# CodeKnight314/Goal-Conditioned-RL-Framework

Measured on AMD Instinct MI355X. Metric: gradient-steps/sec (HER sample + critic+actor update), higher is better.
Workload: dtype f32; 1 GPU; ddpg_pickplace_b256; agent=DDPG, batch_per_gpu=256, buffer_rows=1000000, state_dim=23, action_dim=4, hidden=256, layers=3, k_future=8, gradient_step=40, parallelism=single, hip_graph=True, rng=cpython-mt19937 (host) indices

## Files before the change

### goal-conditioned-rl-framework_amd/_ffi.py

```python
from __future__ import annotations

import ctypes as C
import os

_HERE = os.path.dirname(os.path.abspath(__file__))
LIB_PATH = os.environ.get("GCRL_HIP_LIB") or os.path.join(_HERE, "libgcrl_hip.so")

STREAM_LEGACY = 1
CLONE_AGENT, CLONE_RING = 1, 2
XCHG_HANDLE_BYTES = 256


class GcrlError(RuntimeError):
    pass


class NotEnoughSamples(AssertionError):
    """len(buffer) < batch_size — the reference asserts (src/buffer.py:122)."""


class HerConfig(C.Structure):
    _fields_ = [
        ("state_dim", C.c_int32), ("action_dim", C.c_int32), ("goal_dim", C.c_int32),
        ("capacity", C.c_int64), ("nenvs", C.c_int32), ("k_future", C.c_int32),
# ... 161 lines not shown
    "gcrl_tanh_gauss_bwd_f32": (C.c_int, [_vp, C.c_int, C.c_int, _vp, C.c_int, _vp, _vp, _vp, C.c_int, _f32, C.c_int, C.c_int, _vp, _vp,
                                          C.c_int, _vp]),
    "gcrl_actor_select_f32": (C.c_int, [_vp, _vp, _f32, C.c_int, C.c_int, C.c_int, C.c_int, C.c_int, _f32, _f32, C.c_int, _vp, _vp, _vp, _vp]),
    "gcrl_td3_smooth_f32": (C.c_int, [_vp, C.c_int, C.c_int, C.c_int, _vp, _f32, _f32, _vp]),
    "gcrl_her_set_reward_callback": (C.c_int, [_vp, _vp, _vp]),
    "gcrl_agent_dp_sync_bn": (C.c_int, [_vp, C.c_int, C.c_int, _vp, _vp, _vp]),
    "gcrl_agent_bn_xchg_create": (_vp, [_vp, C.c_int, C.c_int]),
    "gcrl_agent_dp_sync_bn_xchg": (C.c_int, [_vp, C.c_int, C.c_int, _vp]),
    "gcrl_xchg_create": (_vp, [_vp, _i64, _vp, _vp, C.c_int, C.c_int, C.c_int, C.c_int]),
    "gcrl_xchg_destroy": (None, [_vp]),
    "gcrl_xchg_handles": (C.c_int, [_vp, _vp, _i64]),
    "gcrl_xchg_connect": (C.c_int, [_vp, _vp, _i64]),
    "gcrl_xchg_world": (C.c_int, [_vp]),
    "gcrl_xchg_allreduce": (C.c_int, [_vp, C.c_int, C.c_int, _vp]),
    "gcrl_xchg_reset": (C.c_int, [_vp]),
    "gcrl_xchg_selftest": (C.c_int, [_vp, _vp]),
    "gcrl_xchg_read": (C.c_int, [_vp, _i64, _i64, _vp]),
    "gcrl_xchg_get_partials": (C.c_int, [_vp, C.c_int, _vp, C.c_int]),
    "gcrl_agent_xchg_create": (_vp, [_vp, C.c_int, C.c_int]),
    "gcrl_agent_set_exchange": (C.c_int, [_vp, _vp]),
    "gcrl_set_shared_device": (C.c_int, [C.c_int]),
    "gcrl_agent_set_meetings": (C.c_int, [_vp, C.c_int]),
    "gcrl_agent_get_meetings": (C.c_int, [_vp]),
    "gcrl_agent_debug_meet_fault": (C.c_int, [_vp]),
    "gcrl_hash_normal_fill": (C.c_int, [C.c_uint64, C.c_uint64, C.c_int64, _vp, _vp]),
    "gcrl_event_create": (_vp, []),
    "gcrl_event_destroy": (None, [_vp]),
    "gcrl_event_record": (C.c_int, [_vp, _vp]),
    "gcrl_event_elapsed_ms": (C.c_int, [_vp, _vp, C.POINTER(_f32)]),
    "gcrl_stream_synchronize": (C.c_int, [_vp]),
    "gcrl_malloc": (_vp, [C.c_size_t]),
    "gcrl_free": (None, [_vp]),
    "gcrl_memcpy_h2d": (C.c_int, [_vp, _vp, C.c_size_t, _vp]),
    "gcrl_memcpy_d2h": (C.c_int, [_vp, _vp, C.c_size_t, _vp]),
}


def _load():
    if not os.path.exists(LIB_PATH):
        raise ImportError(
            f"{LIB_PATH} is missing: build the HIP extension first "
            "(python -c 'import __graft_entry__ as g; g.build()' or make -C csrc). "
            "There is no CPU fallback.")
    import torch
    lib = C.CDLL(LIB_PATH)
    for name, (res, args) in PROTOTYPES.items():
# ... 43 lines not shown
```

### goal-conditioned-rl-framework_amd/csrc/agent.hip

```cpp
#include <hip/hip_runtime.h>

#include <algorithm>
#include <cmath>
#include <cstdlib>
#include <map>
#include <mutex>
#include <random>
#include <string>
#include <vector>

#include "act_bn.h"
#include "dw_adam.h"
#include "gemm_mfma.h"
#include "her_ring.h"
#include "meet.h"
#include "ops.h"
#include "rowchain.h"
#include "sac_heads.h"
#include "xchg_ipc.h"
#include "pop.h"
#include "pbt_host.h"

using namespace gcrl;

// ... 1948 lines not shown
  for (auto& kv : a->graphs) (void)hipGraphExecDestroy(kv.second);
  a->graphs.clear();
  const gcrl_agent_config& c = a->cfg;
  const bool want = on != 0 && !meet_device_shared();
  a->bn_rsplit = (want && a->bn_slab && a->B > 128 && !std::getenv("GCRL_NO_BN_RSPLIT") && bn_slab_row_split(a->B, a->H, 2) > 1) ? 4 : 1;
  a->rc_merge = want && a->rc_bar && a->split_roles && !std::getenv("GCRL_NO_RC_MERGE") && !std::getenv("GCRL_SPLIT_RG") &&
                rowchain_merge_ok(a->row_rg, a->row_ldl, c.ac_dim, a->H, a->C, a->B);
  a->rc_merge_k = want && a->rc_bar && a->split_k && !std::getenv("GCRL_NO_RC_MERGE");
  a->ddpg_ksplit = want && a->ddpg_ksplit_can && a->rc_bar && !std::getenv("GCRL_NO_DDPG_KSPLIT");
  a->rowtile = want && a->rowtile_can && rowtile_enabled() && rowtile_ok(a->B, a->H, a->L, a->S, a->A, a->C);
  a->opt_fuse = want && a->opt_fuse_can && !std::getenv("GCRL_NO_OPT_FUSE");
  return (a->bn_rsplit > 1 ? 1 : 0) | ((a->rc_merge || a->rc_merge_k || a->ddpg_ksplit) ? 2 : 0) | (a->rowtile ? 4 : 0) | (a->opt_fuse ? 8 : 0);
}

int gcrl_agent_get_meetings(gcrl_agent* a) {
  GCRL_CHECK_ARG(a, "gcrl_agent_get_meetings: null handle");
  if (!meet_device_shared() && meet_probe_device(a->cfg.device)) {
    const int rc = gcrl_agent_set_meetings(a, 0);
    if (rc < 0) return rc;
  }
  return (a->bn_rsplit > 1 ? 1 : 0) | ((a->rc_merge || a->rc_merge_k || a->ddpg_ksplit) ? 2 : 0) | (a->rowtile ? 4 : 0) | (a->opt_fuse ? 8 : 0);
}

int gcrl_agent_debug_meet_fault(gcrl_agent* a) {
  GCRL_CHECK_ARG(a, "gcrl_agent_debug_meet_fault: null handle");
  GCRL_HIP(hipDeviceSynchronize());
  const unsigned long long one = 7;
  float* words = a->rc_merge ? a->rc_bar : (a->bn_rsplit > 1 ? a->bn_bar : nullptr);
  if (a->rowtile) {
    GCRL_HIP(hipMemcpy(a->rt_ctr, &one, sizeof(one), hipMemcpyHostToDevice));
    return GCRL_OK;
  }
  if (a->rc_merge_k || (a->ddpg_ksplit && !a->rowtile)) {
    const unsigned long long far = 1ull << 40;
    GCRL_HIP(hipMemcpy(a->rc_bar + 4, &far, sizeof(far), hipMemcpyHostToDevice));
    return GCRL_OK;
  }
  if (a->opt_fuse) {
    const unsigned int on = 1;
    GCRL_HIP(hipMemcpy(reinterpret_cast<unsigned int*>(a->of_seq) + 1, &on, sizeof(on), hipMemcpyHostToDevice));
    return GCRL_OK;
  }
  GCRL_CHECK_ARG(words, "gcrl_agent_debug_meet_fault: this agent's launches contain no waits (meetings off or not applicable)");
  if (words == a->bn_bar && bn_slab_data_flag()) {
    const unsigned int on = 1;
    GCRL_HIP(hipMemcpy(reinterpret_cast<unsigned int*>(a->bn_bar) + 1, &on, sizeof(on), hipMemcpyHostToDevice));
// ... 314 lines not shown
```

### goal-conditioned-rl-framework_amd/csrc/agent_pop.inc

```

struct gcrl_pop {
  std::vector<gcrl_agent*> m;
  std::map<std::string, void*> tabs;
  std::vector<PopRec> rec;
  long long want[3] = {0, 0, 0}, cap[3] = {0, 0, 0};
  bool no_waits = false;
  int64_t merged = 0, alone = 0;
  bool gather_merge = false;
  int64_t upd_calls = 0, gather_merged = 0, gather_alone = 0;
  PopTabCache act_tabs;
  char *act_blk_host = nullptr, *act_blk_dev = nullptr;
  unsigned long long act_seq = 0;
  char *act_st_host = nullptr, *act_st_dev = nullptr;
  std::vector<int64_t> act_ordered;
  PopProcStep proc;
  int64_t act_calls = 0, act_launches = 0, act_staged = 0;
  PopTabCache clone_tabs;
};

namespace {

constexpr int kMaxPopMembers = 16;
constexpr int kPopActRows = 32;

// ... 319 lines not shown
  };
  const int chunk = std::min(kMaxStepsPerCall, a0->Mmax);
  for (int done = 0; done < n; done += chunk) {
    const int m = std::min(chunk, n - done);
    std::vector<std::vector<StepPlan>> plans(P);
    CallGather cgs[kMaxPopMembers];
    for (int i = 0; i < P; ++i) {
      gcrl_agent* a = p->m[i];
      if (a->wt_dirty) TRY(rc_rebuild_wt(a, st));
      TRY(begin_call_plan(a, rings[i], step0 + done, m, nullptr, 1.0f, st, plans[i], tickets_out ? tickets_out + (size_t)i * n + done : nullptr,
                          tuple_len_out ? tuple_len_out + (size_t)i * n + done : nullptr, false, !tqc || pop_layer_adv(a),
                          &cgs[i]));
    }
    bool one = false;
    TRY(begin_call_issue_pop(p->m.data(), cgs, P, p->gather_merge, st, &one));
    p->upd_calls++;
    if (one) p->gather_merged++;
    else p->gather_alone += P;
    int rc = GCRL_OK;
    for (int i = 0; i < P && !rc; ++i) {
      gcrl_agent* a = p->m[i];
      a->ddpg_ksplit = ksplit; a->opt_fuse = ofuse; a->rowtile = false;
      if (sac) { a->rc_merge = merge; if (!rsplit) a->bn_rsplit = 1; }
      rc = pop_record_steps(a, a0->cap_stream, plans[i], &p->rec[i]);
    }
    restore();
    if (rc) return rc;
    const size_t K = p->rec[0].ops.size();
    for (int i = 1; i < P; ++i)
      if (p->rec[i].ops.size() != K) return fail(GCRL_ERR_STATE, "gcrl_pop_update_n: member %d's step has %zu launches, member 0's %zu", i, p->rec[i].ops.size(), K);
    for (size_t k = 0; k < K; ++k) TRY(pop_issue(p, k, st));
    for (gcrl_agent* a : p->m) TRY(end_call(a, st));
  }
  return GCRL_OK;
}

int gcrl_pop_observe_act(gcrl_pop* p, gcrl_normalizer* const* nz_obs, gcrl_normalizer* const* nz_dg, const float* obs_host, int32_t obs_dim,
                         const float* dg_host, int32_t goal_dim, int32_t n, const double* noise_host, const int32_t* modes, double* out_host,
                         void* stream) {
  GCRL_CHECK_ARG(obs_host, "gcrl_pop_observe_act: obs_host: null array");
  GCRL_CHECK_ARG(dg_host, "gcrl_pop_observe_act: dg_host: null array");
  GCRL_CHECK_ARG(modes, "gcrl_pop_observe_act: modes: null array");
  GCRL_CHECK_ARG(out_host, "gcrl_pop_observe_act: out_host: null array");
  GCRL_CHECK_ARG(modes[0] >= -1 && modes[0] <= 2, "gcrl_pop_observe_act: modes: member 0 has mode %d (-1 skipped, 0, 1 or 2)", modes[0]);
  GCRL_CHECK_ARG(p, "gcrl_pop_observe_act: pop: null handle");
  const int P = (int)p->m.size();
// ... 397 lines not shown
```

### goal-conditioned-rl-framework_amd/csrc/pop.h

```cpp
#pragma once

#include <hip/hip_runtime.h>

#include <atomic>
#include <cstring>
#include <functional>
#include <map>
#include <string>
#include <utility>
#include <vector>

namespace gcrl {

enum PopKind {
  POP_ALONE = 0,
  POP_ROWCHAIN = 1,
  POP_DW_ADAM = 2,
  POP_BEGIN_STEP = 3,
  POP_GEMM_BATCH = 4,
  POP_ADAM = 5,
  POP_ADAM_PAIR = 6,
  POP_BN_FWD = 7,
  POP_BN_BWD = 8,
  POP_BN_BWD_FOLD = 9,
  POP_RC_SPLIT = 10,
  POP_RC_SPLIT_HEADS = 11,
  POP_TG_BWD_SELECT = 12,
  POP_TG_FWD = 13,
  POP_TG_BWD = 14,
};
inline bool pop_mergeable(int kind, int sub) { return kind != POP_ALONE && (kind != POP_GEMM_BATCH || sub == 1); }

struct PopOp {
  int kind = POP_ALONE;
  int sub = 0;
  dim3 grid;
  size_t lds = 0;
  std::vector<char> args;
  std::function<int(hipStream_t)> issue;
};

struct PopRec {
  std::vector<PopOp> ops;
};

PopRec*& pop_rec();
extern std::atomic<int> g_pop_recorders;
inline PopRec* pop_recording() { return g_pop_recorders.load(std::memory_order_relaxed) ? pop_rec() : nullptr; }

inline int pop_record(PopRec* r, int kind, int sub, dim3 grid, size_t lds, const void* args, size_t bytes,
                      std::function<int(hipStream_t)> issue) {
  PopOp op;
  op.kind = kind; op.sub = sub; op.grid = grid; op.lds = lds;
  if (bytes) { op.args.resize(bytes); std::memcpy(op.args.data(), args, bytes); }
  op.issue = std::move(issue);
  r->ops.push_back(std::move(op));
  return 0;
}
inline int pop_defer(PopRec* r, std::function<int(hipStream_t)> issue) {
  return pop_record(r, POP_ALONE, 0, dim3(1), 0, nullptr, 0, std::move(issue));
}

struct PopTabCache {
  std::map<std::string, void*> tabs;
  const std::string* last = nullptr;
  void* last_dev = nullptr;
// ... 45 lines not shown
```

### goal-conditioned-rl-framework_amd/csrc/rowchain.h

```cpp
#pragma once
#include <hip/hip_runtime.h>

#include "gemm_mfma.h"
#include "ops.h"

namespace gcrl {

constexpr int kRowThreads = 256;
constexpr int kRowChunk = 256;

__device__ inline __amdgpu_buffer_rsrc_t bounded_rsrc(const float* p, long long nfloats) {
  const unsigned long long v = (unsigned long long)p;
  const unsigned int lo = __builtin_amdgcn_readfirstlane((unsigned int)v);
  const unsigned int hi = __builtin_amdgcn_readfirstlane((unsigned int)(v >> 32));
  void* q = (void*)(((unsigned long long)hi << 32) | lo);
  const int bytes = __builtin_amdgcn_readfirstlane((int)(nfloats * 4));
  return __builtin_amdgcn_make_buffer_rsrc(q, 0, bytes, 0x00020000);
}

template <int RG>
__device__ __forceinline__ void rows_matmul_wave(const float* xs, int ldx, __amdgpu_buffer_rsrc_t rs, int ldm, int c0,
                                        int jb, int je, v4f (&acc)[RG][4]) {
  const int lane = threadIdx.x & 63;
  constexpr int U = 8;
// ... 14 lines not shown
#pragma unroll
        for (int g = 0; g < RG; ++g) xa[g] = *(const v4f*)(xs + (4 * g + (lane & 3)) * ldx + j + u4);
#pragma unroll
        for (int u = 0; u < 4; ++u)
#pragma unroll
          for (int q = 0; q < 4; ++q)
#pragma unroll
            for (int g = 0; g < RG; ++g)
              acc[g][q] = __builtin_amdgcn_mfma_f32_4x4x1f32(xa[g][u], __uint_as_float(w[u4 + u][q]), acc[g][q], 0, 0, 0);
      }
    }
  };
  v4u wa[U], wb[U];
  load(wa, jb);
  for (int j = jb; j < je; j += 2 * U) {
    load(wb, j + U);
    compute(wa, j);
    load(wa, j + 2 * U);
    compute(wb, j + U);
  }
}

template <int RG>
__device__ __forceinline__ void rows_linear(const float* xs, int ldx, int J, const float* M, int ldm, int N, const float* bias,
                                   int epi, float* part, float* ys, int ldy, float* save, long long ld_save,
                                   int rows_valid, const float* mulH = nullptr, long long ld_mul = 0, int mul = MUL_NONE,
                                   bool chained = false, int pbuf = 0) {
  constexpr int R = 4 * RG;
  const int lane = threadIdx.x & 63;
  const int wave = __builtin_amdgcn_readfirstlane(threadIdx.x >> 6);
  const __amdgpu_buffer_rsrc_t rs = bounded_rsrc(M, (long long)J * ldm);
  const int per = ((J + 3) / 4 + 3) & ~3;
  const int jb = wave * per, je = min(J, jb + per);
  if (chained) {
    part += pbuf * (4 * R * kRowChunk);
    const int pern = ((N + 3) / 4 + 3) & ~3, q4 = pern >> 2;
    const int cb = wave * pern;
    v4f eb[RG], eh[RG];
#pragma unroll
    for (int it = 0; it < RG; ++it) {
      const int idx = lane + 64 * it, r = idx / q4, cc = cb + 4 * (idx - r * q4);
      const bool ok = idx < R * q4 && cc < N;
      eb[it] = (bias && ok) ? *(const v4f*)(bias + cc) : (v4f){0.f, 0.f, 0.f, 0.f};
      eh[it] = (mulH && ok && r < rows_valid) ? *(const v4f*)(mulH + (long long)r * ld_mul + cc) : (v4f){0.f, 0.f, 0.f, 0.f};
    }
    v4f acc[RG][4];
    rows_matmul_wave<RG>(xs, ldx, rs, ldm, 0, jb, je, acc);
#pragma unroll
    for (int g = 0; g < RG; ++g)
#pragma unroll
      for (int i = 0; i < 4; ++i)
        *(v4f*)(part + ((wave * R + 4 * g + i) * kRowChunk) + 4 * lane) =
            (v4f){acc[g][0][i], acc[g][1][i], acc[g][2][i], acc[g][3][i]};
    __syncthreads();
#pragma unroll
    for (int it = 0; it < RG; ++it) {
      const int idx = lane + 64 * it, r = idx / q4, cc = cb + 4 * (idx - r * q4);
      if (idx < R * q4 && cc < N) {
        v4f v = *(const v4f*)(part + r * kRowChunk + cc);
#pragma unroll
        for (int w = 1; w < 4; ++w) v += *(const v4f*)(part + (w * R + r) * kRowChunk + cc);
        v += eb[it];
#pragma unroll
        for (int q = 0; q < 4; ++q) {
          v[q] = act_apply(v[q], epi);
          if (mul != MUL_NONE) v[q] *= act_deriv(eh[it][q], mul);
        }
        *(v4f*)(ys + r * ldy + cc) = v;
        if (save && r < rows_valid) *(v4f*)(save + (long long)r * ld_save + cc) = v;
      }
    }
    return;
  }
  for (int c0 = 0; c0 < N; c0 += kRowChunk) {
    const int c = c0 + 4 * lane;
    v4f b = (v4f){0.f, 0.f, 0.f, 0.f}, hm[RG];
    if (bias && c < N) b = *(const v4f*)(bias + c);
#pragma unroll
    for (int rr = 0; rr < RG; ++rr) {
      const int r = wave + 4 * rr;
      hm[rr] = (mulH && c < N && r < rows_valid) ? *(const v4f*)(mulH + (long long)r * ld_mul + c) : (v4f){0.f, 0.f, 0.f, 0.f};
    }
    v4f acc[RG][4];
    rows_matmul_wave<RG>(xs, ldx, rs, ldm, c0, jb, je, acc);
#pragma unroll
    for (int g = 0; g < RG; ++g)
#pragma unroll
      for (int i = 0; i < 4; ++i)
        *(v4f*)(part + ((wave * R + 4 * g + i) * kRowChunk) + 4 * lane) =
            (v4f){acc[g][0][i], acc[g][1][i], acc[g][2][i], acc[g][3][i]};
    __syncthreads();
    if (c < N) {
#pragma unroll
      for (int rr = 0; rr < RG; ++rr) {
        const int r = wave + 4 * rr;
        v4f v = *(const v4f*)(part + (0 * R + r) * kRowChunk + 4 * lane);
#pragma unroll
        for (int w = 1; w < 4; ++w) v += *(const v4f*)(part + (w * R + r) * kRowChunk + 4 * lane);
        v += b;
#pragma unroll
        for (int q = 0; q < 4; ++q) {
          v[q] = act_apply(v[q], epi);
          if (mul != MUL_NONE) v[q] *= act_deriv(hm[rr][q], mul);
        }
        *(v4f*)(ys + r * ldy + c) = v;
        if (save && r < rows_valid) *(v4f*)(save + (long long)r * ld_save + c) = v;
      }
// ... 47 lines not shown
  const StepCtrl* cur_k; const StepCtrl* cur_p;
  CtrlBlock* cb;
  RowNet actor, tactor, critic[2], tcritic[2];
  int C;
  int target_kind, loss_kind;
  const float* noise; float policy_noise, noise_clamp; unsigned long long seed;
  int given_next, p_critic_only;
  const float* logp_next; float alpha;
  const float* pi;
  const float* sa; const float* nsa; const float* rbuf; const float* dbuf;
  long long slot_x, slot_rd;
  int ldx, ldl, B, S, A, Apad;
  int nblk_k, nblk_p;
  int linear_roles;
  float *hC, *gC, *q, *y, *dq;
  float *hA, *gA, *hC2, *q2, *dz;
  float gamma, clamp_lo;
  unsigned long long* clk;
  float* qt;
  unsigned int* bar;
  unsigned int* status;
  int producers_first;
  int k_split;
};

struct HeadsFold {
  int on;
  int cur_in_k;
  const float* P;
  long long w_mean, b_mean, w_ls, b_ls;
  const float* h_next; const float* h_cur;
  const float* eps_next; const float* eps_cur;
  float* logp_next;
  float* pi; float* logp; float* save_eps; float* save_std; float* head;
  BnRunning run;
};
int launch_rowchain_split(hipStream_t st, const RowChainArgs& a, int rg, int phase, int part, const HeadsFold* hf = nullptr);
bool rowchain_merge_ok(int rg, int ldl, int A, int H, int C, int B);

struct RowActArgs {
  RowNet actor;
  const float* obs; int ld_obs;
  float* out; int ld_out;
  int n, S, A, ldl;
  const double* nz_mean; const double* nz_var; double nz_clip; int D;
  const double* nzg_mean; const double* nzg_var; double nzg_clip;
// ... 20 lines not shown
  unsigned int live, noisy;
  int stride_n;
};
int launch_rowchain_act_pop(hipStream_t st, const RowActPop& c, int members, int n, int ldl, int A, int H);

struct RowTileArgs {
  RowChainArgs rc;
  float* xb;
  float* qpart;
  unsigned long long* ctr;
  unsigned int* xid;
  unsigned int* status;
  int force_sc1;
  int roles[3], nroles, nstage, w16, ldsx, kperx, force_linear, role_mask, sleep_first, sleep_poll;
};
bool rowtile_shape_ok(int B, int H, int L, int S, int A, int C);
bool rowtile_ok(int B, int H, int L, int S, int A, int C);
long long rowtile_ctr_words(int B, int L);
long long rowtile_xb_floats(int B, int H, int L);
long long rowtile_part_floats(int B, int H);
int launch_rowtile_ddpg(hipStream_t st, RowTileArgs t);

int launch_rowchain_ddpg(hipStream_t st, const RowChainArgs& a, int rg);
size_t rowchain_lds_bytes(int rg, int ldl, int A, int H, int C);

int launch_wt_rebuild(hipStream_t st, const RowNet& net, float* Wt);

}
```

### goal-conditioned-rl-framework_amd/csrc/rowchain.hip

```cpp
#include "rowchain.h"
#include "norm_math.h"
#include "meet.h"
#include "sac_select.h"
#include "pop.h"

#include <algorithm>

namespace gcrl {
namespace {

template <int RG>
__device__ inline void load_rows(float* X, int ldl, const float* src, long long ld_src, int ncols, int jpad, int rv) {
  constexpr int R = 4 * RG;
  for (int i = threadIdx.x; i < R * jpad; i += kRowThreads) {
    const int r = i / jpad, c = i - r * jpad;
    X[r * ldl + c] = (r < rv && c < ncols) ? src[(long long)r * ld_src + c] : 0.f;
  }
}

template <int RG>
__device__ inline float* mlp_hidden(const RowNet& net, const float* X0, float* X1, float* X2, int ldl, float* part,
                                    float* save, long long BH, long long row0, int rv, float* last_out = nullptr) {
  const float* in = X0;
  float* out = X1;
  const bool chained = RG == 1 && net.H <= kRowChunk;
  for (int l = 0; l < net.L; ++l) {
    if (last_out && l == net.L - 1) out = last_out;
    rows_linear<RG>(in, ldl, l == 0 ? net.jpad0 : net.H, net.Wt + net.wt[l], net.H, net.H, net.P + net.b[l], EPI_LEAKY,
                    part, out, ldl, save ? save + l * BH + row0 * net.H : nullptr, net.H, rv, nullptr, 0, MUL_NONE,
                    chained, l & 1);
    in = out;
    out = (out == X1) ? X2 : X1;
  }
  if (chained) __syncthreads();
  return (float*)in;
}

template <int RG>
__device__ inline void head_backward(float* h, int ldl, int H, const float* Wh, int n_up, const float* up ,
                                     float* save, int rv, float* q_out = nullptr, float q_bias = 0.f) {
  constexpr int R = 4 * RG;
  const int H4 = H >> 2;
  for (int i = threadIdx.x; i < R * H4; i += kRowThreads) {
    const int r = i / H4, k = (i - r * H4) << 2;
    const v4f hv = *(const v4f*)(h + r * ldl + k);
    v4f s = (v4f){0.f, 0.f, 0.f, 0.f};
    for (int o = 0; o < n_up; ++o) s += up[r * 16 + o] * *(const v4f*)(Wh + (long long)o * H + k);
    v4f g;
#pragma unroll
    for (int q = 0; q < 4; ++q) g[q] = s[q] * act_deriv(hv[q], MUL_DLEAKY);
    if (q_out) {
      const v4f w = *(const v4f*)(Wh + k);
      float qs = ((hv[0] * w[0] + hv[1] * w[1]) + hv[2] * w[2]) + hv[3] * w[3];
// ... 35 lines not shown
#pragma unroll
  for (int u = 0; u < N; ++u) { const int i = threadIdx.x + u * kRowThreads; if (i < n) dst[i] = s.v[u]; }
  for (int i = threadIdx.x + N * kRowThreads; i < n; i += kRowThreads) dst[i] = src[i];
}
template <int RG, int N>
__device__ inline void rows_load(Staged<N>& s, const float* src, long long ld_src, int ncols, int jpad, int rv) {
#pragma unroll
  for (int u = 0; u < N; ++u) {
    const int i = threadIdx.x + u * kRowThreads, r = i / jpad, c = i - r * jpad;
    s.v[u] = (i < 4 * RG * jpad && r < rv && c < ncols) ? src[(long long)r * ld_src + c] : 0.f;
  }
}
template <int RG, int N>
__device__ inline void rows_store(const Staged<N>& s, float* X, int ldl, const float* src, long long ld_src, int ncols, int jpad, int rv) {
#pragma unroll
  for (int u = 0; u < N; ++u) {
    const int i = threadIdx.x + u * kRowThreads, r = i / jpad, c = i - r * jpad;
    if (i < 4 * RG * jpad) X[r * ldl + c] = s.v[u];
  }
  for (int i = threadIdx.x + N * kRowThreads; i < 4 * RG * jpad; i += kRowThreads) {
    const int r = i / jpad, c = i - r * jpad;
    X[r * ldl + c] = (r < rv && c < ncols) ? src[(long long)r * ld_src + c] : 0.f;
  }
}

__device__ inline void stage(float* dst, const float* src, int n) {
  for (int i0 = threadIdx.x; i0 < n; i0 += 8 * kRowThreads) {
    float v[8];
#pragma unroll
    for (int u = 0; u < 8; ++u) { const int i = i0 + u * kRowThreads; v[u] = i < n ? src[i] : 0.f; }
#pragma unroll
    for (int u = 0; u < 8; ++u) { const int i = i0 + u * kRowThreads; if (i < n) dst[i] = v[u]; }
  }
}

template <int RG, bool HF = false>
__device__ __forceinline__ void rowchain_split_body(const RowChainArgs& a, int phase, int part, int bid, const HeadsFold& hfr = HeadsFold{});

template <int RG>
__global__ __launch_bounds__(kRowThreads) void rowchain_ddpg_kernel(RowChainArgs a) {
  kernarg_warm<sizeof(RowChainArgs)>();
#include "rowchain_ddpg_body.inc"
}

template <int RG>
__global__ __launch_bounds__(kRowThreads) void rowchain_ddpg_pop_kernel(const RowChainArgs* __restrict__ tab) {
// ... 428 lines not shown
  const float* rows = c.rows + (size_t)m * c.stride_n * a.ld_obs;
  const double* noise = c.noise + (size_t)m * c.stride_n * a.A;
  double* out = c.out + (size_t)m * c.stride_n * a.A;
  rowchain_act_body<true>(a, [&](long long i) { return __hip_atomic_load(rows + i, __ATOMIC_RELAXED, __HIP_MEMORY_SCOPE_SYSTEM); },
                          [&](long long t) { return __hip_atomic_load(noise + t, __ATOMIC_RELAXED, __HIP_MEMORY_SCOPE_SYSTEM); },
                          ((c.noisy >> m) & 1u) != 0, out, lds);
  asm volatile("s_waitcnt vmcnt(0)" ::: "memory");
  __syncthreads();
  if (threadIdx.x == 0 && c.flags) __hip_atomic_store(c.flags + (size_t)m * gridDim.x + blockIdx.x, c.seq, __ATOMIC_RELAXED, __HIP_MEMORY_SCOPE_SYSTEM);
}

__global__ void wt_rebuild_kernel(RowNet net, float* Wt) {
  const int l = blockIdx.y;
  const int in = l == 0 ? net.in : net.H, J = l == 0 ? net.jpad0 : net.H, H = net.H;
  const long long n = (long long)J * H;
  for (long long i = (long long)blockIdx.x * blockDim.x + threadIdx.x; i < n; i += (long long)gridDim.x * blockDim.x) {
    const int k = (int)(i / H), o = (int)(i - (long long)k * H);
    Wt[net.wt[l] + i] = k < in ? net.P[net.w[l] + (long long)o * in + k] : 0.f;
  }
}

}

size_t rowchain_lds_bytes(int rg, int ldl, int A, int H, int C) {
  const int R = 4 * rg;
  return (size_t)(4 * R * ldl + (rg == 1 ? 2 : 1) * 4 * R * kRowChunk + 4 * R * 16 + std::max(std::max(2 * A + 1, A + 2 * C), C * (A + 1)) * H + 96) * sizeof(float);
}

bool rowchain_merge_ok(int rg, int ldl, int A, int H, int C, int B) {
  const size_t lds = rowchain_lds_bytes(rg, ldl, A, H, C);
  if (lds > 160 * 1024) return false;
  const void* k = rg == 1 ? (const void*)rowchain_split_kernel<1> : (rg == 2 ? (const void*)rowchain_split_kernel<2> : (const void*)rowchain_split_kernel<4>);
  if (lds > 64 * 1024 && hipFuncSetAttribute(k, hipFuncAttributeMaxDynamicSharedMemorySize, (int)lds) != hipSuccess) return false;
  const long long nblk = (B + 4 * rg - 1) / (4 * rg);
  const void* kh = rg == 1 ? (const void*)rowchain_split_heads_kernel<1> : (rg == 2 ? (const void*)rowchain_split_heads_kernel<2> : (const void*)rowchain_split_heads_kernel<4>);
  if (lds > 64 * 1024 && hipFuncSetAttribute(kh, hipFuncAttributeMaxDynamicSharedMemorySize, (int)lds) != hipSuccess) return false;
  return 2LL * C * nblk <= meet_capacity(k, kRowThreads, lds) && 2LL * C * nblk <= meet_capacity(kh, kRowThreads, lds);
}

int launch_rowchain_ddpg(hipStream_t st, const RowChainArgs& a, int rg) {
  GCRL_CHECK_ARG(rg == 1 || rg == 2 || rg == 4, "rowchain: rows per block must be 4, 8 or 16");
  GCRL_CHECK_ARG(a.critic[0].H % 4 == 0 && a.ldl % 4 == 0 && a.A <= 16 && a.C >= 1 && a.C <= 2,
                 "rowchain: unsupported shape (H=%d, A=%d, C=%d)", a.critic[0].H, a.A, a.C);
  const size_t lds = rowchain_lds_bytes(rg, a.ldl, a.A, a.critic[0].H, a.C);
  GCRL_CHECK_ARG(lds <= 160 * 1024, "rowchain: %zu bytes of LDS needed", lds);
  GCRL_CHECK_ARG(!a.k_split || (a.bar && a.qt && a.producers_first && a.C == 1), "rowchain: the two-role critic phase needs its meeting counters");
  const int grid = (a.k_split ? 2 : 1) * a.nblk_k + a.nblk_p;
  if (grid < 1) return GCRL_OK;
  if (PopRec* r = pop_recording())
    return pop_record(r, POP_ROWCHAIN, rg, dim3(grid), lds, &a, sizeof(a), [ac = a, rg](hipStream_t s) { return launch_rowchain_ddpg(s, ac, rg); });
  auto go = [&](auto kern) -> int {
    static thread_local size_t raised = 0;
    if (lds > 64 * 1024 && lds > raised) {
      GCRL_HIP(hipFuncSetAttribute((const void*)kern, hipFuncAttributeMaxDynamicSharedMemorySize, (int)lds));
      raised = lds;
    }
    hipLaunchKernelGGL(kern, dim3(grid), dim3(kRowThreads), lds, st, a);
    GCRL_HIP(hipGetLastError());
    return GCRL_OK;
  };
  if (rg == 1) return go(rowchain_ddpg_kernel<1>);
  if (rg == 2) return go(rowchain_ddpg_kernel<2>);
  return go(rowchain_ddpg_kernel<4>);
}

int launch_rowchain_split(hipStream_t st, const RowChainArgs& a, int rg, int phase, int part, const HeadsFold* hf) {
  GCRL_CHECK_ARG(rg == 1 || rg == 2 || rg == 4, "rowchain: rows per block must be 4, 8 or 16");
  GCRL_CHECK_ARG(a.critic[0].H % 4 == 0 && a.ldl % 4 == 0 && a.A <= 16 && a.C >= 1 && a.C <= 2 && (phase == 0 || phase == 1) &&
                     (part >= 1 && part <= 3) && (part != 3 || a.bar) && (phase == 0 || a.p_critic_only) && a.qt,
                 "rowchain split: unsupported shape (H=%d, A=%d, C=%d, phase %d part %d)", a.critic[0].H, a.A, a.C, phase, part);
  const size_t lds = rowchain_lds_bytes(rg, a.ldl, a.A, a.critic[0].H, a.C);
  GCRL_CHECK_ARG(lds <= 160 * 1024, "rowchain: %zu bytes of LDS needed", lds);
  const int nblk = (a.B + 4 * rg - 1) / (4 * rg);
// ... 154 lines not shown
```

### goal-conditioned-rl-framework_amd/csrc/rowchain_ddpg_body.inc

```
  extern __shared__ __attribute__((aligned(16))) float lds[];
  if (a.k_split && a.nblk_k) {
    if ((int)blockIdx.x < 2 * a.nblk_k) {
      if (a.clk && threadIdx.x == 0 && blockIdx.x == 0) atomicMin(&a.clk[0], (unsigned long long)wall_clock64());
      rowchain_split_body<RG>(a, 0, 3, (int)blockIdx.x);
      if (a.clk && threadIdx.x == 0) atomicMax(&a.clk[1], (unsigned long long)wall_clock64());
      return;
    }
  }
  const int kblocks = (a.k_split && a.nblk_k) ? 2 * a.nblk_k : a.nblk_k;
  constexpr int R = 4 * RG;
  const int ldl = a.ldl, H = a.critic[0].H, S = a.S, A = a.A, B = a.B;
  float* X0 = lds;
  float* X1 = X0 + R * ldl;
  float* X2 = X1 + R * ldl;
  float* XS = X2 + R * ldl;
  float* part = XS + R * ldl;
  float* sm = part + R * 16 + (RG == 1 ? 2 : 1) * 4 * R * kRowChunk;
  float* sm2 = sm + R * 16;
  float* sm3 = sm2 + R * 16;
  float* hw = sm3 + R * 16;
  float* hb = hw + max(max(2 * A + 1, A + 2 * a.C), a.C * (A + 1)) * H;
  bool role_k = (int)blockIdx.x < kblocks;
  int blk = role_k ? (int)blockIdx.x : (int)blockIdx.x - kblocks;
  if (a.nblk_k == a.nblk_p && (a.nblk_k & 3) == 0 && !a.linear_roles && !a.k_split) {
// ... 142 lines not shown
      if (r < rv) { a.q2[row0 + r] = q0; if (C > 1) a.q2[(long long)B + row0 + r] = q1; }
    }
    __syncthreads();
    for (int k = 0; k < C; ++k) {
      const float* hs = a.hC2 + (long long)k * a.critic[k].L * BH;
      const float* hsrc = hs + (a.critic[k].L - 1) * BH + row0 * H;
      for (int i = tid; i < R * H; i += kRowThreads) {
        const int r = i / H, kk = i - r * H;
        XS[r * ldl + kk] = r < rv ? hsrc[(long long)r * H + kk] : 0.f;
      }
      __syncthreads();
      head_backward<RG>(XS, ldl, H, hw_c + k * H, 1, sm2 + k, nullptr, rv);
      __syncthreads();
      float* g0 = grad_chain<RG>(a.critic[k], XS, X1, X2, ldl, part + R * 16, hs, nullptr, BH, row0, rv);
      rows_head<RG>(g0, ldl, H, hw_da + k * A * H, H, nullptr, A, EPI_NONE, sm);
      __syncthreads();
      if (tid < R * A) {
        const int r = tid / A, o = tid - r * A;
        if (r < rv) a.dz[((long long)k * B + row0 + r) * a.Apad + o] = sm[r * 16 + o];
      }
      __syncthreads();
    }
  } else {
    const StepCtrl c = *a.cur_p;
    const float* sa_rows = a.sa + (long long)c.batch_slot * a.slot_x + row0 * a.ldx;
    constexpr int NX = 2 * RG;
    const int jp_s = max(a.actor.jpad0, a.critic[0].jpad0);
    float* hw_a = hw; float* hw_c = hw + A * H; float* hw_da = hw_c + H;
    const float* src_a = a.actor.P + a.actor.w[a.actor.L];
    const float* src_c = a.critic[0].P + a.critic[0].w[a.critic[0].L];
    const float* src_da = a.critic[0].Wt + a.critic[0].wt[0] + (long long)S * H;
    Staged<NX> s_s;
    rows_load<RG>(s_s, sa_rows, a.ldx, S, jp_s, rv);
    Staged<8> s_a, s_hc, s_da;
    seg_load(s_a, src_a, A * H);
    seg_load(s_hc, src_c, H);
    seg_load(s_da, src_da, A * H);
    float v_hb = 0.f;
    if (tid < A) v_hb = a.actor.P[a.actor.b[a.actor.L] + tid];
    if (tid == 32) v_hb = a.critic[0].P[a.critic[0].b[a.critic[0].L]];
    rows_store<RG>(s_s, X0, ldl, sa_rows, a.ldx, S, jp_s, rv);
    seg_store(s_a, hw_a, src_a, A * H);
    seg_store(s_hc, hw_c, src_c, H);
    seg_store(s_da, hw_da, src_da, A * H);
    if (tid < A) hb[tid] = v_hb;
    if (tid == 32) hb[16] = v_hb;
    const bool fuse_q = head_fusable(H);
    if (fuse_q && tid < R) sm2[tid * 16] = (tid < rv) ? -1.0f / (float)B : 0.f;
    __syncthreads();
    float* h = mlp_hidden<RG>(a.actor, X0, X1, X2, ldl, part + R * 16, a.hA, BH, row0, rv, XS);
    rows_head<RG>(h, ldl, H, hw_a, H, hb, A, EPI_TANH, sm);
    __syncthreads();
    if (tid < R * A) { const int r = tid / A, o = tid - r * A; X0[r * ldl + S + o] = sm[r * 16 + o]; }
    __syncthreads();
    h = mlp_hidden<RG>(a.critic[0], X0, X1, X2, ldl, part + R * 16, a.hC2, BH, row0, rv);
    if (fuse_q) {
      head_backward<RG>(h, ldl, H, hw_c, 1, sm2, nullptr, rv, sm3, hb[16]);
      __syncthreads();
      if (tid < rv) a.q2[row0 + tid] = sm3[tid * 16];
    } else {
      rows_head<RG>(h, ldl, H, hw_c, H, hb + 16, 1, EPI_NONE, sm2);
      __syncthreads();
      if (tid < R) {
        if (tid < rv) a.q2[row0 + tid] = sm2[tid * 16];
        sm2[tid * 16] = (tid < rv) ? -1.0f / (float)B : 0.f;
      }
      __syncthreads();
      head_backward<RG>(h, ldl, H, hw_c, 1, sm2, nullptr, rv);
      __syncthreads();
    }
    float* g0 = grad_chain<RG>(a.critic[0], h, X1, X2, ldl, part + R * 16, a.hC2, nullptr, BH, row0, rv);
    rows_head<RG>(g0, ldl, H, hw_da, H, nullptr, A, EPI_NONE, sm2);
    __syncthreads();
    if (tid < R * A) {
      const int r = tid / A, o = tid - r * A;
      const float act = sm[r * 16 + o];
      const float g = sm2[r * 16 + o] * act_deriv(act, MUL_DTANH);
      sm2[r * 16 + o] = g;
// ... 9 lines not shown
```

### include/gcrl.h

```cpp
#ifndef GCRL_H
#define GCRL_H

#include <stddef.h>
#include <stdint.h>

#ifdef __cplusplus
extern "C" {
#endif

#define GCRL_ABI_VERSION 1
#define GCRL_STREAM_LEGACY ((void*)1)

typedef enum gcrl_status {
  GCRL_OK = 0,
  GCRL_ERR_ARG = -1,
  GCRL_ERR_HIP = -2,
  GCRL_ERR_NOT_ENOUGH = -3,
  GCRL_ERR_STATE = -4
} gcrl_status;

const char* gcrl_last_error(void);
int gcrl_abi_version(void);
int gcrl_device_count(void);

// ... 206 lines not shown
#define GCRL_XCHG_HANDLE_BYTES 256
typedef struct gcrl_xchg gcrl_xchg;
gcrl_xchg* gcrl_xchg_create(float* arena_dev, int64_t arena_floats, const int64_t* seg_off, const int64_t* seg_n, int nseg, int rank,
                            int world, int device);
void gcrl_xchg_destroy(gcrl_xchg* x);
int gcrl_xchg_handles(gcrl_xchg* x, uint8_t* out, int64_t n);
int gcrl_xchg_connect(gcrl_xchg* x, const uint8_t* all_ranks_records, int64_t n);
int gcrl_xchg_world(const gcrl_xchg* x);
int gcrl_xchg_allreduce(gcrl_xchg* x, int seg0, int nseg, void* stream);
int gcrl_xchg_get_partials(gcrl_xchg* x, int seg, float* out_host, int n);
int gcrl_xchg_read(gcrl_xchg* x, int64_t first, int64_t n, float* out_host);
int gcrl_xchg_selftest(gcrl_xchg* x, void* stream);
int gcrl_xchg_reset(gcrl_xchg* x);
gcrl_xchg* gcrl_agent_xchg_create(gcrl_agent* a, int rank, int world);
int gcrl_agent_set_exchange(gcrl_agent* a, gcrl_xchg* x);
int gcrl_agent_dp_run_all(gcrl_agent* a, gcrl_dp* d, void* stream);
typedef int (*gcrl_exchange_fn)(float* buf_dev, int64_t n, void* stream, void* user);
int gcrl_agent_dp_sync_bn(gcrl_agent* a, int world, int rank, gcrl_dp* dp, gcrl_exchange_fn fn, void* user);
gcrl_xchg* gcrl_agent_bn_xchg_create(gcrl_agent* a, int rank, int world);
int gcrl_agent_dp_sync_bn_xchg(gcrl_agent* a, int world, int rank, gcrl_xchg* bx);
int gcrl_set_shared_device(int shared);
int gcrl_agent_set_meetings(gcrl_agent* a, int on);
int gcrl_agent_get_meetings(gcrl_agent* a);
int gcrl_agent_debug_meet_fault(gcrl_agent* a);
int gcrl_agent_dev_ptr(gcrl_agent* a, const char* name, float** ptr_dev_out, int64_t* numel_out);

int gcrl_agent_act(gcrl_agent* a, const float* obs_dev, int n, int ld_obs, float* out_dev,
                   int ld_out, const float* eps_dev, void* stream);
int gcrl_agent_act_host(gcrl_agent* a, const float* obs_host, int n, int ld_obs, float* out_host,
                        int ld_out, void* stream);

typedef struct gcrl_normalizer gcrl_normalizer;
gcrl_normalizer* gcrl_normalizer_create(int size, double clip_range, double eps, int device);
void gcrl_normalizer_destroy(gcrl_normalizer* z);
int gcrl_normalizer_size(const gcrl_normalizer* z);
int gcrl_normalizer_update(gcrl_normalizer* z, const float* x, int n, int ld, int on_device, void* stream);
int gcrl_normalizer_normalize(gcrl_normalizer* z, const float* x, int n, int ld, int on_device, float* out, int ld_out,
                              int out_on_device, void* stream);
int gcrl_normalizer_get(gcrl_normalizer* z, double* mean_host, double* var_host, double* count_host);
int gcrl_normalizer_set(gcrl_normalizer* z, const double* mean_host, const double* var_host, double count, double clip_range);
int gcrl_normalizer_set_float32(gcrl_normalizer* z, int on);
int gcrl_normalizer_is_float32(const gcrl_normalizer* z);
int gcrl_normalizer_set_rows_float64(gcrl_normalizer* z, int on);
int gcrl_agent_observe_act(gcrl_agent* a, gcrl_normalizer* nz_obs, gcrl_normalizer* nz_dg, const float* obs_host, int obs_dim,
                           const float* dg_host, int goal_dim, int n, const double* noise_host, int mode, double* out_host,
                           void* stream);
// ... 69 lines not shown
```

Before: 19320 gradient-steps/s.

## Stage first-layer actor and critic weights in LDS and pre-accumulate critic state part

```diff
diff --git a/goal-conditioned-rl-framework_amd/_ffi.py b/goal-conditioned-rl-framework_amd/_ffi.py
--- a/goal-conditioned-rl-framework_amd/_ffi.py
+++ b/goal-conditioned-rl-framework_amd/_ffi.py
@@ -207,6 +207,7 @@
     "gcrl_set_shared_device": (C.c_int, [C.c_int]),
     "gcrl_agent_set_meetings": (C.c_int, [_vp, C.c_int]),
     "gcrl_agent_get_meetings": (C.c_int, [_vp]),
+    "gcrl_rowchain_l0_forms": (C.c_int, [C.POINTER(_i64), C.POINTER(_i64)]),
     "gcrl_agent_debug_meet_fault": (C.c_int, [_vp]),
     "gcrl_hash_normal_fill": (C.c_int, [C.c_uint64, C.c_uint64, C.c_int64, _vp, _vp]),
     "gcrl_event_create": (_vp, []),
diff --git a/goal-conditioned-rl-framework_amd/csrc/agent.hip b/goal-conditioned-rl-framework_amd/csrc/agent.hip
--- a/goal-conditioned-rl-framework_amd/csrc/agent.hip
+++ b/goal-conditioned-rl-framework_amd/csrc/agent.hip
@@ -1994,6 +1994,14 @@
   return (a->bn_rsplit > 1 ? 1 : 0) | ((a->rc_merge || a->rc_merge_k || a->ddpg_ksplit) ? 2 : 0) | (a->rowtile ? 4 : 0) | (a->opt_fuse ? 8 : 0);
 }
 
+int gcrl_rowchain_l0_forms(int64_t* lds_form_out, int64_t* stream_form_out) {
+  GCRL_CHECK_ARG(lds_form_out && stream_form_out, "gcrl_rowchain_l0_forms: null output");
+  long long l = 0, s = 0;
+  rowchain_l0_counts(&l, &s);
+  *lds_form_out = l; *stream_form_out = s;
+  return GCRL_OK;
+}
+
 int gcrl_agent_debug_meet_fault(gcrl_agent* a) {
   GCRL_CHECK_ARG(a, "gcrl_agent_debug_meet_fault: null handle");
   GCRL_HIP(hipDeviceSynchronize());
diff --git a/goal-conditioned-rl-framework_amd/csrc/agent_pop.inc b/goal-conditioned-rl-framework_amd/csrc/agent_pop.inc
--- a/goal-conditioned-rl-framework_amd/csrc/agent_pop.inc
+++ b/goal-conditioned-rl-framework_amd/csrc/agent_pop.inc
@@ -365,6 +365,7 @@
       gcrl_agent* a = p->m[i];
       a->ddpg_ksplit = ksplit; a->opt_fuse = ofuse; a->rowtile = false;
       if (sac) { a->rc_merge = merge; if (!rsplit) a->bn_rsplit = 1; }
+      p->rec[i].members = P;
       rc = pop_record_steps(a, a0->cap_stream, plans[i], &p->rec[i]);
     }
     restore();
diff --git a/goal-conditioned-rl-framework_amd/csrc/pop.h b/goal-conditioned-rl-framework_amd/csrc/pop.h
--- a/goal-conditioned-rl-framework_amd/csrc/pop.h
+++ b/goal-conditioned-rl-framework_amd/csrc/pop.h
@@ -42,6 +42,7 @@
 
 struct PopRec {
   std::vector<PopOp> ops;
+  int members = 1;
 };
 
 PopRec*& pop_rec();
diff --git a/goal-conditioned-rl-framework_amd/csrc/rowchain.h b/goal-conditioned-rl-framework_amd/csrc/rowchain.h
--- a/goal-conditioned-rl-framework_amd/csrc/rowchain.h
+++ b/goal-conditioned-rl-framework_amd/csrc/rowchain.h
@@ -60,10 +60,63 @@
 }
 
 template <int RG>
+__device__ __forceinline__ void rows_matmul_wave_lds(const float* xs, int ldx, const float* ml, int ldm, int c0, int jb, int je,
+                                                     int kb, int ke, v4f (&acc)[RG][4]) {
+  const int lane = threadIdx.x & 63;
+  const float* wp = ml + min(c0 + 4 * lane, ldm - 4);
+  for (int j = jb; j < je; j += 4) {
+    if (j + 4 <= kb || j >= ke) continue;
+    v4f xa[RG];
+#pragma unroll
+    for (int g = 0; g < RG; ++g) xa[g] = *(const v4f*)(xs + (4 * g + (lane & 3)) * ldx + j);
+#pragma unroll
+    for (int u = 0; u < 4; ++u) {
+      if (j + u >= kb && j + u < ke) {
+        const v4f w = *(const v4f*)(wp + (j + u) * ldm);
+#pragma unroll
+        for (int q = 0; q < 4; ++q)
+#pragma unroll
+          for (int g = 0; g < RG; ++g) acc[g][q] = __builtin_amdgcn_mfma_f32_4x4x1f32(xa[g][u], w[q], acc[g][q], 0, 0, 0);
+      }
+    }
+  }
+}
+
+__device__ __forceinline__ void rows_share(int J, int& jb, int& je) {
+  const int wave = __builtin_amdgcn_readfirstlane(threadIdx.x >> 6);
+  const int per = ((J + 3) / 4 + 3) & ~3;
+  jb = wave * per; je = min(J, jb + per);
+}
+
+template <int RG>
+struct RowsCarry { v4f acc[RG][4]; };
+template <int RG>
+__device__ __forceinline__ void rows_linear_begin(const float* xs, int ldx, int J, const float* ml, int ldm, int kcut, RowsCarry<RG>& carry) {
+#pragma unroll
+  for (int g = 0; g < RG; ++g)
+#pragma unroll
+    for (int q = 0; q < 4; ++q) carry.acc[g][q] = (v4f){0.f, 0.f, 0.f, 0.f};
+  int jb, je;
+  rows_share(J, jb, je);
+  rows_matmul_wave_lds<RG>(xs, ldx, ml, ldm, 0, jb, je, jb, min(je, kcut), carry.acc);
+}
+
+template <int RG>
+__device__ __forceinline__ void rows_matmul_lds_rest(const float* xs, int ldx, const float* ml, int ldm, int jb, int je, int kcut,
+                                                     const RowsCarry<RG>* carry, v4f (&acc)[RG][4]) {
+#pragma unroll
+  for (int g = 0; g < RG; ++g)
+#pragma unroll
+    for (int q = 0; q < 4; ++q) acc[g][q] = carry ? carry->acc[g][q] : (v4f){0.f, 0.f, 0.f, 0.f};
+  rows_matmul_wave_lds<RG>(xs, ldx, ml, ldm, 0, jb, je, carry ? max(jb, kcut) : jb, je, acc);
+}
+
+template <int RG>
 __device__ __forceinline__ void rows_linear(const float* xs, int ldx, int J, const float* M, int ldm, int N, const float* bias,
                                    int epi, float* part, float* ys, int ldy, float* save, long long ld_save,
                                    int rows_valid, const float* mulH = nullptr, long long ld_mul = 0, int mul = MUL_NONE,
-                                   bool chained = false, int pbuf = 0) {
+                                   bool chained = false, int pbuf = 0, const float* ml = nullptr, int kcut = 0,
+                                   const RowsCarry<RG>* carry = nullptr) {
   constexpr int R = 4 * RG;
   const int lane = threadIdx.x & 63;
   const int wave = __builtin_amdgcn_readfirstlane(threadIdx.x >> 6);
@@ -83,7 +136,8 @@
       eh[it] = (mulH && ok && r < rows_valid) ? *(const v4f*)(mulH + (long long)r * ld_mul + cc) : (v4f){0.f, 0.f, 0.f, 0.f};
     }
     v4f acc[RG][4];
-    rows_matmul_wave<RG>(xs, ldx, rs, ldm, 0, jb, je, acc);
+    if (ml) rows_matmul_lds_rest<RG>(xs, ldx, ml, ldm, jb, je, kcut, carry, acc);
+    else rows_matmul_wave<RG>(xs, ldx, rs, ldm, 0, jb, je, acc);
 #pragma unroll
     for (int g = 0; g < RG; ++g)
 #pragma unroll
@@ -120,7 +174,8 @@
       hm[rr] = (mulH && c < N && r < rows_valid) ? *(const v4f*)(mulH + (long long)r * ld_mul + c) : (v4f){0.f, 0.f, 0.f, 0.f};
     }
     v4f acc[RG][4];
-    rows_matmul_wave<RG>(xs, ldx, rs, ldm, c0, jb, je, acc);
+    if (ml) rows_matmul_lds_rest<RG>(xs, ldx, ml, ldm, jb, je, kcut, carry, acc);
+    else rows_matmul_wave<RG>(xs, ldx, rs, ldm, c0, jb, je, acc);
 #pragma unroll
     for (int g = 0; g < RG; ++g)
 #pragma unroll
@@ -214,6 +269,7 @@
   unsigned int* status;
   int producers_first;
   int k_split;
+  int l0_lds;
 };
 
 struct HeadsFold {
@@ -280,7 +336,8 @@
 int launch_rowtile_ddpg(hipStream_t st, RowTileArgs t);
 
 int launch_rowchain_ddpg(hipStream_t st, const RowChainArgs& a, int rg);
-size_t rowchain_lds_bytes(int rg, int ldl, int A, int H, int C);
+size_t rowchain_lds_bytes(int rg, int ldl, int A, int H, int C, long long l0_floats = 0);
+void rowchain_l0_counts(long long* lds_form, long long* stream_form);
 
 int launch_wt_rebuild(hipStream_t st, const RowNet& net, float* Wt);
 
diff --git a/goal-conditioned-rl-framework_amd/csrc/rowchain.hip b/goal-conditioned-rl-framework_amd/csrc/rowchain.hip
--- a/goal-conditioned-rl-framework_amd/csrc/rowchain.hip
+++ b/goal-conditioned-rl-framework_amd/csrc/rowchain.hip
@@ -5,6 +5,8 @@
 #include "pop.h"
 
 #include <algorithm>
+#include <atomic>
+#include <cstdlib>
 
 namespace gcrl {
 namespace {
@@ -20,15 +22,16 @@
 
 template <int RG>
 __device__ inline float* mlp_hidden(const RowNet& net, const float* X0, float* X1, float* X2, int ldl, float* part,
-                                    float* save, long long BH, long long row0, int rv, float* last_out = nullptr) {
+                                    float* save, long long BH, long long row0, int rv, float* last_out = nullptr,
+                                    const float* ml0 = nullptr, int first = 0) {
   const float* in = X0;
-  float* out = X1;
+  float* out = (first & 1) ? X2 : X1;
   const bool chained = RG == 1 && net.H <= kRowChunk;
-  for (int l = 0; l < net.L; ++l) {
+  for (int l = first; l < net.L; ++l) {
     if (last_out && l == net.L - 1) out = last_out;
     rows_linear<RG>(in, ldl, l == 0 ? net.jpad0 : net.H, net.Wt + net.wt[l], net.H, net.H, net.P + net.b[l], EPI_LEAKY,
                     part, out, ldl, save ? save + l * BH + row0 * net.H : nullptr, net.H, rv, nullptr, 0, MUL_NONE,
-                    chained, l & 1);
+                    chained, l & 1, l == 0 ? ml0 : nullptr);
     in = out;
     out = (out == X1) ? X2 : X1;
   }
@@ -110,6 +113,20 @@
     const int r = i / jpad, c = i - r * jpad;
     X[r * ldl + c] = (r < rv && c < ncols) ? src[(long long)r * ld_src + c] : 0.f;
   }
+}
+
+template <int N>
+struct Staged4 { v4f v[N]; };
+template <int N>
+__device__ __forceinline__ void img_load(Staged4<N>& s, const float* src, int n4) {
+#pragma unroll
+  for (int u = 0; u < N; ++u) { const int i = threadIdx.x + u * kRowThreads; s.v[u] = i < n4 ? ((const v4f*)src)[i] : (v4f){0.f, 0.f, 0.f, 0.f}; }
+}
+template <int N>
+__device__ __forceinline__ void img_store(const Staged4<N>& s, float* dst, const float* src, int n4) {
+#pragma unroll
+  for (int u = 0; u < N; ++u) { const int i = threadIdx.x + u * kRowThreads; if (i < n4) ((v4f*)dst)[i] = s.v[u]; }
+  for (int i = threadIdx.x + N * kRowThreads; i < n4; i += kRowThreads) ((v4f*)dst)[i] = ((const v4f*)src)[i];
 }
 
 __device__ inline void stage(float* dst, const float* src, int n) {
@@ -584,10 +601,26 @@
 
 }
 
-size_t rowchain_lds_bytes(int rg, int ldl, int A, int H, int C) {
+size_t rowchain_lds_bytes(int rg, int ldl, int A, int H, int C, long long l0_floats) {
   const int R = 4 * rg;
-  return (size_t)(4 * R * ldl + (rg == 1 ? 2 : 1) * 4 * R * kRowChunk + 4 * R * 16 + std::max(std::max(2 * A + 1, A + 2 * C), C * (A + 1)) * H + 96) * sizeof(float);
-}
+  return (size_t)(4 * R * ldl + (rg == 1 ? 2 : 1) * 4 * R * kRowChunk + 4 * R * 16 + std::max(std::max(2 * A + 1, A + 2 * C), C * (A + 1)) * H + 96 + l0_floats) * sizeof(float);
+}
+
+namespace {
+std::atomic<long long> g_l0_lds_launches{0}, g_l0_stream_launches{0};
+long long rowchain_l0_floats(const RowChainArgs& a, int rg, int grid, int members) {
+  static const bool off = [] { const char* e = std::getenv("GCRL_ROW_L0_LDS"); return e && e[0] == '0'; }();
+  const int H = a.critic[0].H;
+  if (off || rg > 2 || a.nblk_p < 1 || a.p_critic_only || H > kRowChunk || a.actor.H != H) return 0;
+  const long long fl = (long long)(a.actor.jpad0 + a.critic[0].jpad0) * H;
+  const size_t kLds = 160 * 1024, was = rowchain_lds_bytes(rg, a.ldl, a.A, H, a.C), now = rowchain_lds_bytes(rg, a.ldl, a.A, H, a.C, fl);
+  if (now > kLds) return 0;
+  if (kLds / now == kLds / was) return fl;
+  static const int cus = [] { int dev = 0, n = 0; if (hipGetDevice(&dev) != hipSuccess || hipDeviceGetAttribute(&n, hipDeviceAttributeMultiprocessorCount, dev) != hipSuccess) n = 0; return n; }();
+  return (long long)grid * members <= (long long)cus * (long long)(kLds / now) ? fl : 0;
+}
+}
+void rowchain_l0_counts(long long* lds_form, long long* stream_form) { *lds_form = g_l0_lds_launches.load(); *stream_form = g_l0_stream_launches.load(); }
 
 bool rowchain_merge_ok(int rg, int ldl, int A, int H, int C, int B) {
   const size_t lds = rowchain_lds_bytes(rg, ldl, A, H, C);
@@ -600,17 +633,22 @@
   return 2LL * C * nblk <= meet_capacity(k, kRowThreads, lds) && 2LL * C * nblk <= meet_capacity(kh, kRowThreads, lds);
 }
 
-int launch_rowchain_ddpg(hipStream_t st, const RowChainArgs& a, int rg) {
+int launch_rowchain_ddpg(hipStream_t st, const RowChainArgs& args, int rg) {
   GCRL_CHECK_ARG(rg == 1 || rg == 2 || rg == 4, "rowchain: rows per block must be 4, 8 or 16");
-  GCRL_CHECK_ARG(a.critic[0].H % 4 == 0 && a.ldl % 4 == 0 && a.A <= 16 && a.C >= 1 && a.C <= 2,
-                 "rowchain: unsupported shape (H=%d, A=%d, C=%d)", a.critic[0].H, a.A, a.C);
-  const size_t lds = rowchain_lds_bytes(rg, a.ldl, a.A, a.critic[0].H, a.C);
+  GCRL_CHECK_ARG(args.critic[0].H % 4 == 0 && args.ldl % 4 == 0 && args.A <= 16 && args.C >= 1 && args.C <= 2,
+                 "rowchain: unsupported shape (H=%d, A=%d, C=%d)", args.critic[0].H, args.A, args.C);
+  GCRL_CHECK_ARG(!args.k_split || (args.bar && args.qt && args.producers_first && args.C == 1), "rowchain: the two-role critic phase needs its meeting counters");
+  const int grid = (args.k_split ? 2 : 1) * args.nblk_k + args.nblk_p;
+  if (grid < 1) return GCRL_OK;
+  PopRec* const rec = pop_recording();
+  const long long l0_floats = rowchain_l0_floats(args, rg, grid, rec ? std::max(rec->members, 1) : 1);
+  RowChainArgs a = args;
+  a.l0_lds = l0_floats ? 1 : 0;
+  const size_t lds = rowchain_lds_bytes(rg, a.ldl, a.A, a.critic[0].H, a.C, l0_floats);
   GCRL_CHECK_ARG(lds <= 160 * 1024, "rowchain: %zu bytes of LDS needed", lds);
-  GCRL_CHECK_ARG(!a.k_split || (a.bar && a.qt && a.producers_first && a.C == 1), "rowchain: the two-role critic phase needs its meeting counters");
-  const int grid = (a.k_split ? 2 : 1) * a.nblk_k + a.nblk_p;
-  if (grid < 1) return GCRL_OK;
-  if (PopRec* r = pop_recording())
-    return pop_record(r, POP_ROWCHAIN, rg, dim3(grid), lds, &a, sizeof(a), [ac = a, rg](hipStream_t s) { return launch_rowchain_ddpg(s, ac, rg); });
+  if (a.nblk_p >= 1 && !a.p_critic_only) (l0_floats ? g_l0_lds_launches : g_l0_stream_launches).fetch_add(1, std::memory_order_relaxed);
+  if (PopRec* r = rec)
+    return pop_record(r, POP_ROWCHAIN, rg, dim3(grid), lds, &a, sizeof(a), [ac = args, rg](hipStream_t s) { return launch_rowchain_ddpg(s, ac, rg); });
   auto go = [&](auto kern) -> int {
     static thread_local size_t raised = 0;
     if (lds > 64 * 1024 && lds > raised) {
diff --git a/goal-conditioned-rl-framework_amd/csrc/rowchain_ddpg_body.inc b/goal-conditioned-rl-framework_amd/csrc/rowchain_ddpg_body.inc
--- a/goal-conditioned-rl-framework_amd/csrc/rowchain_ddpg_body.inc
+++ b/goal-conditioned-rl-framework_amd/csrc/rowchain_ddpg_body.inc
@@ -188,6 +188,15 @@
       __syncthreads();
     }
   } else {
+    const bool l0 = RG <= 2 && a.l0_lds != 0;
+    float* wl_a = hb + 96; float* wl_c = wl_a + a.actor.jpad0 * H;
+    const float* src_la = a.actor.Wt + a.actor.wt[0];
+    const float* src_lc = a.critic[0].Wt + a.critic[0].wt[0];
+    const int n4_la = l0 ? (a.actor.jpad0 * H) >> 2 : 0, n4_lc = l0 ? (a.critic[0].jpad0 * H) >> 2 : 0;
+    Staged4<8> s_la, s_lc;
+    img_load(s_la, src_la, n4_la);
+    img_load(s_lc, src_lc, n4_lc);
+    asm volatile("" ::: "memory");
     const StepCtrl c = *a.cur_p;
     const float* sa_rows = a.sa + (long long)c.batch_slot * a.slot_x + row0 * a.ldx;
     constexpr int NX = 2 * RG;
@@ -211,15 +220,21 @@
     seg_store(s_da, hw_da, src_da, A * H);
     if (tid < A) hb[tid] = v_hb;
     if (tid == 32) hb[16] = v_hb;
+    img_store(s_la, wl_a, src_la, n4_la);
+    img_store(s_lc, wl_c, src_lc, n4_lc);
     const bool fuse_q = head_fusable(H);
     if (fuse_q && tid < R) sm2[tid * 16] = (tid < rv) ? -1.0f / (float)B : 0.f;
     __syncthreads();
-    float* h = mlp_hidden<RG>(a.actor, X0, X1, X2, ldl, part + R * 16, a.hA, BH, row0, rv, XS);
+    RowsCarry<RG> c0acc;
+    if (l0) rows_linear_begin<RG>(X0, ldl, a.critic[0].jpad0, wl_c, H, S, c0acc);
+    float* h = mlp_hidden<RG>(a.actor, X0, X1, X2, ldl, part + R * 16, a.hA, BH, row0, rv, XS, l0 ? wl_a : nullptr);
     rows_head<RG>(h, ldl, H, hw_a, H, hb, A, EPI_TANH, sm);
     __syncthreads();
     if (tid < R * A) { const int r = tid / A, o = tid - r * A; X0[r * ldl + S + o] = sm[r * 16 + o]; }
     __syncthreads();
-    h = mlp_hidden<RG>(a.critic[0], X0, X1, X2, ldl, part + R * 16, a.hC2, BH, row0, rv);
+    rows_linear<RG>(X0, ldl, a.critic[0].jpad0, src_lc, H, H, a.critic[0].P + a.critic[0].b[0], EPI_LEAKY, part + R * 16, X1, ldl,
+                    a.hC2 + row0 * H, H, rv, nullptr, 0, MUL_NONE, RG == 1 && H <= kRowChunk, 0, l0 ? wl_c : nullptr, S, &c0acc);
+    h = mlp_hidden<RG>(a.critic[0], X1, X1, X2, ldl, part + R * 16, a.hC2, BH, row0, rv, nullptr, nullptr, 1);
     if (fuse_q) {
       head_backward<RG>(h, ldl, H, hw_c, 1, sm2, nullptr, rv, sm3, hb[16]);
       __syncthreads();
diff --git a/include/gcrl.h b/include/gcrl.h
--- a/include/gcrl.h
+++ b/include/gcrl.h
@@ -252,6 +252,7 @@
 int gcrl_set_shared_device(int shared);
 int gcrl_agent_set_meetings(gcrl_agent* a, int on);
 int gcrl_agent_get_meetings(gcrl_agent* a);
+int gcrl_rowchain_l0_forms(int64_t* lds_form_out, int64_t* stream_form_out);
 int gcrl_agent_debug_meet_fault(gcrl_agent* a);
 int gcrl_agent_dev_ptr(gcrl_agent* a, const char* name, float** ptr_dev_out, int64_t* numel_out);
 
```

Result: slower. 18450 gradient-steps/s (-4.5%).
